# mosure/bevy_gaussian_splatting

Hardware: NVIDIA H100
Metric: rendered Msplats/sec @1080p, 6M-gaussian cloud (higher is better)
Workload: dtype f32 (f16-packed inputs)

## Files before the change

### bevy_gaussian_splatting_b200/csrc/project.cu

```cuda
#include <cuda_fp16.h>

#include "project_math.cuh"
#include "launch.cuh"

namespace bgs {

__constant__ float c_shc[16] = {
    0.28209479177387814f, -0.4886025119029199f, 0.4886025119029199f, -0.4886025119029199f,
    1.0925484305920792f, -1.0925484305920792f, 0.31539156525252005f, -1.0925484305920792f,
    0.5462742152960396f, -0.5900435899266435f, 2.890611442640554f, -0.4570457994644658f,
    0.3731763325901154f, -0.4570457994644658f, 1.445305721320277f, -0.5900435899266435f};

__device__ __forceinline__ void normalize3(const float a[3], float out[3]) {
    const float inv = rsqrtf((a[0] * a[0] + a[1] * a[1]) + a[2] * a[2]);
    out[0] = a[0] * inv; out[1] = a[1] * inv; out[2] = a[2] * inv;
}
__device__ __forceinline__ float dot3(const float a[3], const float b[3]) {
    return (a[0] * b[0] + a[1] * b[1]) + a[2] * b[2];
}
__device__ __forceinline__ float srgb_to_linear(float v) {
    if (v <= 0.04045f) return v * (1.0f / 12.92f);
    return __powf((v + 0.055f) * (1.0f / 1.055f), 2.4f);
}
__device__ __forceinline__ uint32_t pack_bbox(float lo, float hi) {
    return (uint32_t)(int)lo | ((uint32_t)(int)hi << 16);
}
constexpr uint32_t BBOX_EMPTY = 1u;

__device__ __forceinline__ void make_bbox(float cx, float cy, float hx, float hy, int Wi, int Hi,
                                          uint32_t& bx, uint32_t& by) {
    bx = BBOX_EMPTY; by = BBOX_EMPTY;
    if (!(hx >= 0.0f) || !(hy >= 0.0f) || !(cx == cx) || !(cy == cy)) return;
    const float sx = hx * 1.0e-3f + 1.0e-2f, sy = hy * 1.0e-3f + 1.0e-2f;
    float x0 = ceilf((cx - hx) - (0.5f + sx));
    float x1 = floorf((cx + hx) - (0.5f - sx));
    float y0 = ceilf((cy - hy) - (0.5f + sy));
    float y1 = floorf((cy + hy) - (0.5f - sy));
    if (!(x0 <= x1) || !(y0 <= y1)) return;
    x0 = fmaxf(x0, 0.0f); y0 = fmaxf(y0, 0.0f);
    x1 = fminf(x1, (float)(Wi - 1)); y1 = fminf(y1, (float)(Hi - 1));
    if (!(x0 <= x1) || !(y0 <= y1)) return;
    bx = pack_bbox(x0, x1); by = pack_bbox(y0, y1);
}

template <bool F16>
struct Attr;
template <>
struct Attr<false> {
    __device__ static float4 load(const void* blocks, uint32_t id, float* sh, float q[4], float so[4], bool need_sh,
                                  uint32_t* = nullptr) {
        const float4* b = reinterpret_cast<const float4*>(blocks) + (size_t)id * 16;
        const float4 p = __ldg(b), r = __ldg(b + 1), s = __ldg(b + 2);
        q[0] = r.x; q[1] = r.y; q[2] = r.z; q[3] = r.w;
        so[0] = s.x; so[1] = s.y; so[2] = s.z; so[3] = s.w;
        if (need_sh) {
#pragma unroll
            for (int i = 0; i < 12; ++i) {
                const float4 v = __ldg(b + 3 + i);
                sh[4 * i] = v.x; sh[4 * i + 1] = v.y; sh[4 * i + 2] = v.z; sh[4 * i + 3] = v.w;
            }
        }
        return p;
    }
};
template <>
struct Attr<true> {
    __device__ static float lo(uint32_t w) { return __half2float(__ushort_as_half((unsigned short)(w & 0xFFFFu))); }
    __device__ static float hi(uint32_t w) { return __half2float(__ushort_as_half((unsigned short)(w >> 16))); }
    __device__ static float4 load(const void* blocks, uint32_t id, float* sh, float q[4], float so[4], bool need_sh,
                                  uint32_t* op_bits = nullptr) {
        const uint4* b = reinterpret_cast<const uint4*>(blocks) + (size_t)id * 8;
        const uint4 pw = __ldg(b), w = __ldg(b + 1);
        if (op_bits) *op_bits = w.w & 0xFFFFu;
        q[0] = hi(w.x); q[1] = lo(w.x); q[2] = hi(w.y); q[3] = lo(w.y);
        so[0] = hi(w.z); so[1] = lo(w.z); so[2] = hi(w.w); so[3] = lo(w.w);
        if (need_sh) {
#pragma unroll
            for (int i = 0; i < 6; ++i) {
                const uint4 v = __ldg(b + 2 + i);
                sh[8 * i] = lo(v.x); sh[8 * i + 1] = hi(v.x); sh[8 * i + 2] = lo(v.y); sh[8 * i + 3] = hi(v.y);
                sh[8 * i + 4] = lo(v.z); sh[8 * i + 5] = hi(v.z); sh[8 * i + 6] = lo(v.w); sh[8 * i + 7] = hi(v.w);
            }
        }
        return make_float4(__uint_as_float(pw.x), __uint_as_float(pw.y), __uint_as_float(pw.z), __uint_as_float(pw.w));
    }
};

template <bool F16>
__global__ void repack_kernel(const uint4* __restrict__ pos, const uint4* __restrict__ sh, const uint4* __restrict__ rot,
                              const uint4* __restrict__ so, uint32_t n, uint4* __restrict__ blocks) {
    constexpr uint32_t CH = F16 ? 8u : 16u;
    constexpr uint32_t SHC = F16 ? 6u : 12u;
    const size_t i = (size_t)blockIdx.x * blockDim.x + threadIdx.x;
    if (i >= (size_t)n * CH) return;
    const uint32_t id = (uint32_t)(i / CH), c = (uint32_t)(i % CH);
    uint4 v = make_uint4(0u, 0u, 0u, 0u);
    if (c == 0) v = pos[id];
    else if (c == 1) v = rot[id];
    else if (!F16 && c == 2) v = so[id];
    else {
        const uint32_t k = c - (F16 ? 2u : 3u);
        if (k < SHC) v = sh[(size_t)id * SHC + k];
    }
    blocks[i] = v;
}
void launch_repack(bool f16, const void* pos, const void* sh, const void* rot, const void* so, uint32_t n, void* blocks,
                   cudaStream_t stream) {
    const size_t total = (size_t)n * (f16 ? 8 : 16);
    const uint32_t grid = (uint32_t)((total + 255) / 256);
    if (f16) repack_kernel<true><<<grid, 256, 0, stream>>>((const uint4*)pos, (const uint4*)sh, (const uint4*)rot, (const uint4*)so, n, (uint4*)blocks);
    else repack_kernel<false><<<grid, 256, 0, stream>>>((const uint4*)pos, (const uint4*)sh, (const uint4*)rot, (const uint4*)so, n, (uint4*)blocks);
}

__global__ void depth_range_kernel(const float4* __restrict__ pos, uint32_t n, const uint32_t* __restrict__ sorted_payload,
                                   const uint32_t* __restrict__ slot_ids ,
                                   FrameCounters* __restrict__ ctr, FrameConsts fc) {
    if (threadIdx.x != 0 || blockIdx.x != 0 || n < 2u) return;
    const uint32_t n_vis = ctr->n_vis, n_sorted = ctr->n_sort;
    auto id_at = [&](uint32_t i) { const uint32_t p = sorted_payload[i]; return slot_ids ? slot_ids[p] : p; };
    uint32_t first, last;
    if (n_sorted == n) {
        first = id_at(1u); last = id_at(n - 1u);
    } else {
        const uint32_t cmin = 0xFFFFFFFFu - ctr->culled_min_inv, cmax = ctr->culled_max_p1 - 1u;
        first = n_vis >= 2u ? id_at(1u) : cmin;
        last = (n - n_vis) >= 1u ? cmax : id_at(n - 1u);
    }
    auto dist = [&](uint32_t id) {
        const float4 p = pos[id];
        float pw[4];
        mat4_point(fc.model, p.x, p.y, p.z, pw);
        return sqrtf(cam_dist2(fc, pw));
    };
    ctr->depth_min = dist(last);
    ctr->depth_max = dist(first);
}

__device__ __forceinline__ float adaptive_cutoff(float opacity) {
    const float a = 9.0f + 2.0f * det_ln(opacity);
    return sqrtf(a > 0.000001f ? a : 0.000001f);
}
__global__ void cutoff_table_kernel(float* __restrict__ tab) {
    const uint32_t h = blockIdx.x * blockDim.x + threadIdx.x;
    if (h < 65536u) tab[h] = adaptive_cutoff(__half2float(__ushort_as_half((unsigned short)h)));
}
void launch_cutoff_table(float* tab, cudaStream_t stream) { cutoff_table_kernel<<<256, 256, 0, stream>>>(tab); }

template <bool F16>
__device__ __forceinline__ float splat_cutoff(const FrameConsts& fc, float opacity, const float* __restrict__ cutoff_tab,
                                              uint32_t op_bits) {
    if (!fc.adaptive) return 3.0f;
    if constexpr (F16) return __ldg(cutoff_tab + op_bits);
    else return adaptive_cutoff(opacity);
}

__device__ __forceinline__ void rotation_rows(const float q[4], float Rm[3][3]) {
    const float qr = q[0], x = q[1], y = q[2], z = q[3];
    Rm[0][0] = 1.0f - 2.0f * (y * y + z * z);
    Rm[1][0] = 2.0f * (x * y - qr * z);
    Rm[2][0] = 2.0f * (x * z + qr * y);
    Rm[0][1] = 2.0f * (x * y + qr * z);
    Rm[1][1] = 1.0f - 2.0f * (x * x + z * z);
    Rm[2][1] = 2.0f * (y * z - qr * x);
    Rm[0][2] = 2.0f * (x * z - qr * y);
    Rm[1][2] = 2.0f * (y * z + qr * x);
    Rm[2][2] = 1.0f - 2.0f * (x * x + y * y);
}

__device__ __forceinline__ void sigma3d(const FrameConsts& fc, const float A[3][3], const float Rm[3][3], const float sc[3],
                                        const float q[4], const float so[4], float c3[6]) {
    if (fc.cov_pre) {
        c3[0] = q[0]; c3[1] = q[1]; c3[2] = q[2]; c3[3] = q[3]; c3[4] = so[0]; c3[5] = so[1];
        return;
    }
    float M[3][3], Sg[3][3], X[3][3], TS[3][3];
#pragma unroll
    for (int i = 0; i < 3; ++i)
#pragma unroll
        for (int j = 0; j < 3; ++j) M[i][j] = sc[i] * Rm[i][j];
#pragma unroll
    for (int i = 0; i < 3; ++i)
#pragma unroll
        for (int j = 0; j < 3; ++j) Sg[i][j] = (M[0][i] * M[0][j] + M[1][i] * M[1][j]) + M[2][i] * M[2][j];
    const float mn = fminf(fminf(fminf(fabsf(Sg[0][0]), fabsf(Sg[0][1])), fminf(fabsf(Sg[0][2]), fabsf(Sg[1][1]))),
                           fminf(fabsf(Sg[1][2]), fabsf(Sg[2][2])));
    const float mx = fmaxf(fmaxf(fmaxf(fabsf(Sg[0][0]), fabsf(Sg[0][1])), fmaxf(fabsf(Sg[0][2]), fabsf(Sg[1][1]))),
                           fmaxf(fabsf(Sg[1][2]), fabsf(Sg[2][2])));
    if (fc.model_identity && mn > 0.0f && mx < __uint_as_float(0x7F800000u) && Sg[0][0] == Sg[0][0] &&
        Sg[0][1] == Sg[0][1] && Sg[0][2] == Sg[0][2] && Sg[1][1] == Sg[1][1] && Sg[1][2] == Sg[1][2] && Sg[2][2] == Sg[2][2]) {
#pragma unroll
        for (int i = 0; i < 3; ++i)
#pragma unroll
            for (int j = 0; j < 3; ++j) TS[i][j] = Sg[i][j];
    } else {
#pragma unroll
        for (int i = 0; i < 3; ++i)
#pragma unroll
            for (int j = 0; j < 3; ++j) X[i][j] = (A[i][0] * Sg[0][j] + A[i][1] * Sg[1][j]) + A[i][2] * Sg[2][j];
#pragma unroll
        for (int i = 0; i < 3; ++i)
#pragma unroll
            for (int j = 0; j < 3; ++j) TS[i][j] = (X[i][0] * A[j][0] + X[i][1] * A[j][1]) + X[i][2] * A[j][2];
    }
    c3[0] = TS[0][0]; c3[1] = TS[1][0]; c3[2] = TS[2][0]; c3[3] = TS[1][1]; c3[4] = TS[2][1]; c3[5] = TS[2][2];
}

struct Cov2d {
    float a, b, c, det, mid, term, l1;
};
__device__ __forceinline__ Cov2d cov2d(const FrameConsts& fc, const float pw[3], const float c3[6]) {
    const float Vrk[3][3] = {{c3[0], c3[1], c3[2]}, {c3[1], c3[3], c3[4]}, {c3[2], c3[4], c3[5]}};
    float tv[4];
    mat4_point(fc.view_from_world, pw[0], pw[1], pw[2], tv);
    const float fx = fc.p00 * fc.W, fy = fc.p11 * fc.H;
    const float sz = 1.0f / (tv[2] * tv[2]);
    const float J00 = fx / tv[2], J20 = -(fx * tv[0]) * sz;
    const float J11 = -fy / tv[2], J21 = (fy * tv[1]) * sz;
    float Tm[3][2];
#pragma unroll
    for (int i = 0; i < 3; ++i) {
        const float v0 = fc.view_from_world[i * 4 + 0], v1 = fc.view_from_world[i * 4 + 1],
                    v2 = fc.view_from_world[i * 4 + 2];
        Tm[i][0] = v0 * J00 + v2 * J20;
        Tm[i][1] = v1 * J11 + v2 * J21;
    }
    float Y[3][2];
#pragma unroll
    for (int i = 0; i < 3; ++i)
#pragma unroll
        for (int b = 0; b < 2; ++b) Y[i][b] = (Vrk[i][0] * Tm[0][b] + Vrk[i][1] * Tm[1][b]) + Vrk[i][2] * Tm[2][b];
    Cov2d v;
    v.a = ((Tm[0][0] * Y[0][0] + Tm[1][0] * Y[1][0]) + Tm[2][0] * Y[2][0]) + 0.3f;
    v.b = (Tm[0][1] * Y[0][0] + Tm[1][1] * Y[1][0]) + Tm[2][1] * Y[2][0];
    v.c = ((Tm[0][1] * Y[0][1] + Tm[1][1] * Y[1][1]) + Tm[2][1] * Y[2][1]) + 0.3f;
    v.det = v.a * v.c - v.b * v.b;
    v.mid = 0.5f * (v.a + v.c);
    v.term = sqrtf(fmaxf(0.0f, v.mid * v.mid - v.det));
    v.l1 = v.mid + v.term;
    return v;
}

__device__ __forceinline__ void aabb_record(const FrameConsts& fc, const Cov2d& v, float cutoff, SplatRec& rec) {
    const float l2 = fmaxf(v.mid - v.term, 0.0f);
    const float Rq = cutoff * fmaxf(sqrtf(v.l1), sqrtf(l2));
    const float dinv = 1.0f / v.det;
    rec.ux = v.c * dinv; rec.uy = -v.b * dinv; rec.vx = v.a * dinv; rec.vy = Rq;
    const float h = 0.5f * Rq;
    make_bbox(rec.cx, rec.cy, h, h, fc.Wi, fc.Hi, rec.bx, rec.by);
}

__device__ __forceinline__ void obb_record(const FrameConsts& fc, const Cov2d& v, float cutoff, SplatRec& rec) {
    const float a = v.a, b = v.b, c = v.c;
    const float aa = (a - c) * (a - c);
    const float bb = sqrtf(aa + (4.0f * b) * b);
    const float major = sqrtf(((a + c) + bb) * 0.5f);
    const float minor = sqrtf(((a + c) - bb) * 0.5f);
    const float Bx = cutoff * major, By = cutoff * minor;
    const float evx = -b, evy = v.l1 - a;
    const float el = sqrtf(evx * evx + evy * evy);
    const float e1x = evx / el, e1y = evy / el;
    const float e2x = e1y, e2y = -e1x;
    rec.ux = (2.0f * e1x) / Bx; rec.uy = (-2.0f * e1y) / Bx;
    rec.vx = (2.0f * e2x) / By; rec.vy = (-2.0f * e2y) / By;
    const float hx = 0.5f * (fabsf(e1x) * Bx + fabsf(e2x) * By);
    const float hy = 0.5f * (fabsf(e1y) * Bx + fabsf(e2y) * By);
    if (rec.ux == rec.ux && rec.uy == rec.uy && rec.vx == rec.vx && rec.vy == rec.vy)
        make_bbox(rec.cx, rec.cy, hx, hy, fc.Wi, fc.Hi, rec.bx, rec.by);
}

__device__ __forceinline__ void surfel_record(const FrameConsts& fc, const float A[3][3], const float Rm[3][3],
                                              const float sc[3], const float pw[3], float cutoff, uint32_t r,
                                              float4* __restrict__ extra, SplatRec& rec) {
    const float W = fc.W, H = fc.H;
    float L[3][2];
#pragma unroll
    for (int j = 0; j < 2; ++j) {
        const float rc[3] = {Rm[j][0] * sc[j], Rm[j][1] * sc[j], Rm[j][2] * sc[j]};
#pragma unroll
        for (int i = 0; i < 3; ++i) L[i][j] = (A[i][0] * rc[0] + A[i][1] * rc[1]) + A[i][2] * rc[2];
    }
    float G[3][4];
    mat4_dir(fc.clip_from_world, L[0][0], L[1][0], L[2][0], G[0]);
    mat4_dir(fc.clip_from_world, L[0][1], L[1][1], L[2][1], G[1]);
    mat4_point(fc.clip_from_world, pw[0], pw[1], pw[2], G[2]);
    const float fxk = fc.p00 * W / 2.0f, fyk = fc.p11 * H / 2.0f;
    const float cxk = (W - 1.0f) / 2.0f, cyk = (H - 1.0f) / 2.0f;
    float T0[3], T1[3], T2[3];
#pragma unroll
    for (int j = 0; j < 3; ++j) {
        T0[j] = fxk * G[j][0] + cxk * G[j][3];
        T1[j] = fyk * G[j][1] + cyk * G[j][3];
        T2[j] = G[j][3];
    }
    const float c2 = cutoff * cutoff;
    const float test[3] = {c2, c2, -1.0f};
    const float tt[3] = {test[0] * T2[0], test[1] * T2[1], test[2] * T2[2]};
    const float d = dot3(tt, T2);
    if (fabsf(d) < 1.0e-4f) return;
    const float inv = 1.0f / d;
    const float f[3] = {inv * test[0], inv * test[1], inv * test[2]};
    const float t02[3] = {T0[0] * T2[0], T0[1] * T2[1], T0[2] * T2[2]};
    const float t12[3] = {T1[0] * T2[0], T1[1] * T2[1], T1[2] * T2[2]};
    const float mean0 = dot3(f, t02), mean1 = dot3(f, t12);
    const float f0[3] = {f[0] * T0[0], f[1] * T0[1], f[2] * T0[2]};
    const float f1[3] = {f[0] * T1[0], f[1] * T1[1], f[2] * T1[2]};
    const float ex = mean0 * mean0 - dot3(f0, T0);
    const float ey = mean1 * mean1 - dot3(f1, T1);
    if (ex < 1.0e-4f || ey < 1.0e-4f) return;
    const float Rq = fmaxf(fmaxf(sqrtf(ex), sqrtf(ey)), cutoff * 0.707106f);
    rec.ux = 2.0f / Rq; rec.uy = 0.0f; rec.vx = 0.0f; rec.vy = -2.0f / Rq;
    const float h = 0.5f * Rq;
    if (Rq == Rq) make_bbox(rec.cx, rec.cy, h, h, fc.Wi, fc.Hi, rec.bx, rec.by);
    if (fc.aabb && extra != nullptr) {
        float4* e = extra + (size_t)r * 4;
        e[0] = make_float4(Rq, mean0, mean1, W / H);
        e[1] = make_float4(T0[0], T0[1], T0[2], 0.0f);
        e[2] = make_float4(T1[0], T1[1], T1[2], 0.0f);
        e[3] = make_float4(T2[0], T2[1], T2[2], 0.0f);
    }
}

__device__ __forceinline__ void sh_colour(const FrameConsts& fc, const float A[3][3], const float pw[3], const float sh[48],
                                          float rgb[3]) {
    const float dlt[3] = {pw[0] - fc.cam[0], pw[1] - fc.cam[1], pw[2] - fc.cam[2]};
    float dw[3], loc[3], dl[3];
    normalize3(dlt, dw);
    if (fc.model_identity) {
        loc[0] = dw[0]; loc[1] = dw[1]; loc[2] = dw[2];
    } else {
#pragma unroll
        for (int cc = 0; cc < 3; ++cc) {
            const float col[3] = {A[0][cc], A[1][cc], A[2][cc]};
            float bn[3];
            normalize3(col, bn);
            loc[cc] = dot3(bn, dw);
        }
    }
    normalize3(loc, dl);
    const float x = dl[0], y = dl[1], z = dl[2];
    const float xx = x * x, yy = y * y, zz = z * z;
    float basis[16];
    basis[0] = 1.0f;
    basis[1] = y; basis[2] = z; basis[3] = x;
    basis[4] = x * y; basis[5] = y * z; basis[6] = (2.0f * zz - xx) - yy;
    basis[7] = x * z; basis[8] = xx - yy;
    basis[9] = y * (3.0f * xx - yy);
    basis[10] = (x * y) * z;
    basis[11] = y * ((4.0f * zz - xx) - yy);
    basis[12] = z * ((2.0f * zz - 3.0f * xx) - 3.0f * yy);
    basis[13] = x * ((4.0f * zz - xx) - yy);
    basis[14] = z * (xx - yy);
    basis[15] = x * (xx - 3.0f * yy);
#pragma unroll
    for (int kk = 0; kk < 16; ++kk) basis[kk] *= c_shc[kk];
#pragma unroll
    for (int cc = 0; cc < 3; ++cc) {
        float acc = 0.5f;
#pragma unroll
        for (int kk = 0; kk < 16; ++kk) acc = fmaf(sh[3 * kk + cc], basis[kk], acc);
        rgb[cc] = acc;
    }
    if (fc.color_space == 0u) {
#pragma unroll
        for (int cc = 0; cc < 3; ++cc) rgb[cc] = srgb_to_linear(rgb[cc]);
    }
}

__device__ __forceinline__ void depth_colour(const FrameConsts& fc, const FrameCounters* __restrict__ ctr,
                                             const float pw[3], float rgb[3]) {
    if (fc.n_cloud < 2u) return;
    const float depth = sqrtf(cam_dist2(fc, pw));
    const float dmin = ctr->depth_min, dmax = ctr->depth_max;
    float nd = (depth - dmin) / (dmax - dmin);
    nd = fminf(fmaxf(nd, 0.0f), 1.0f);
    float t1 = (nd - 0.5f) / (1.0f - 0.5f); t1 = fminf(fmaxf(t1, 0.0f), 1.0f);
    float t2 = (nd - 0.0f) / (0.5f - 0.0f); t2 = fminf(fmaxf(t2, 0.0f), 1.0f);
    rgb[0] = t1 * t1 * (3.0f - 2.0f * t1);
    rgb[1] = 1.0f - fabsf(nd - 0.5f) * 2.0f;
    rgb[2] = 1.0f - t2 * t2 * (3.0f - 2.0f * t2);
}

__device__ __forceinline__ void normal_colour(const FrameConsts& fc, const float A[3][3], const float Rm[3][3],
                                              const float sc[3], float rgb[3]) {
    float SR[3], Ln[3], wn[4];
#pragma unroll
    for (int i = 0; i < 3; ++i) SR[i] = sc[i] * Rm[i][2];
#pragma unroll
    for (int i = 0; i < 3; ++i) Ln[i] = (A[i][0] * SR[0] + A[i][1] * SR[1]) + A[i][2] * SR[2];
    mat4_dir(fc.view_from_world, Ln[0], Ln[1], Ln[2], wn);
    const float l = sqrtf(((wn[0] * wn[0] + wn[1] * wn[1]) + wn[2] * wn[2]) + wn[3] * wn[3]);
#pragma unroll
    for (int cc = 0; cc < 3; ++cc) rgb[cc] = 0.5f * (wn[cc] / l + 1.0f);
}

__device__ __forceinline__ void position_colour(const FrameConsts& fc, const float pw[3], float rgb[3]) {
#pragma unroll
    for (int cc = 0; cc < 3; ++cc) rgb[cc] = (pw[cc] - fc.aabb_min[cc]) / (fc.aabb_max[cc] - fc.aabb_min[cc]);
}

constexpr float FRAC_PI_3_F = 1.0471975512f;
constexpr float PI_2_F = 6.28318530718f;

__device__ __forceinline__ void hsv_to_rgb(float h, float s, float v, float rgb[3]) {
    const float hk = h / FRAC_PI_3_F, vs = v * s;
    const float base[3] = {5.0f, 3.0f, 1.0f};
#pragma unroll
    for (int cc = 0; cc < 3; ++cc) {
        const float x = base[cc] + hk;
        const float k = x - 6.0f * truncf(x / 6.0f);
        rgb[cc] = v - vs * fmaxf(0.0f, fminf(k, fminf(4.0f - k, 1.0f)));
    }
}

__device__ __forceinline__ float det_atan2(float yf, float xf) {
    if (yf != yf || xf != xf) return __uint_as_float(0x7FC00000u);
    const double ay = fabs((double)yf), ax = fabs((double)xf);
    const bool steep = ay > ax;
    double t;
    if (ax == ay) t = ax == 0.0 ? 0.0 : 1.0;
    else t = steep ? __ddiv_rn(ax, ay) : __ddiv_rn(ay, ax);
    double base = 0.0, u = t;
    if (t > 0.41421356237309503) { base = 0.7853981633974483; u = __ddiv_rn(__dsub_rn(t, 1.0), __dadd_rn(t, 1.0)); }
    const double z = __dmul_rn(u, u);
    double p = -1.0 / 43.0;
#pragma unroll
    for (int k = 20; k >= 0; --k) p = __dadd_rn(__dmul_rn(p, z), (k & 1 ? -1.0 : 1.0) / (double)(2 * k + 1));
    double r = __dadd_rn(base, __dmul_rn(u, p));
    if (steep) r = __dsub_rn(1.5707963267948966, r);
    if (__float_as_uint(xf) >> 31) r = __dsub_rn(3.141592653589793, r);
    if (__float_as_uint(yf) >> 31) r = -r;
    return (float)r;
}

__device__ __forceinline__ void class_colour(const ModeConsts& mc, float vis, float rgb[3]) {
    if (vis < 2.0f) return;
    const float hue = ((vis - 2.0f) / (float)mc.num_classes) * 6.283185307f;
    float h[3];
    hsv_to_rgb(hue, 1.0f, 1.0f, h);
#pragma unroll
    for (int cc = 0; cc < 3; ++cc) rgb[cc] = rgb[cc] * (1.0f - 0.5f) + h[cc] * 0.5f;
}

__device__ __forceinline__ void flow_colour(const FrameConsts& fc, const ModeConsts& mc, const float pw[3], float rgb[3]) {
    float c[4], cp[4];
    mat4_point(fc.clip_from_world, pw[0], pw[1], pw[2], c);
    mat4_point(mc.prev_clip_from_world, pw[0], pw[1], pw[2], cp);
    const float mvx = (c[0] / c[3] - cp[0] / cp[3]) * 0.5f;
    const float mvy = (c[1] / c[3] - cp[1] / cp[3]) * -0.5f;
    const float fx = mvx / mc.delta_time, fy = mvy / mc.delta_time;
    const float radius = sqrtf(fx * fx + fy * fy);
    float angle = det_atan2(fy, fx);
    if (angle < 0.0f) angle = angle + PI_2_F;
    hsv_to_rgb(angle, fminf(fmaxf(radius, 0.0f), 1.0f), 1.0f, rgb);
}

__device__ __forceinline__ void highlight_selected(SplatRec& rec, float drgb[3], float nrgb[3]) {
    rec.r = 0.3f; rec.g = 1.0f; rec.b = 0.1f; rec.op = 1.0f;
    drgb[0] = nrgb[0] = 0.3f; drgb[1] = nrgb[1] = 1.0f; drgb[2] = nrgb[2] = 0.1f;
}

__device__ __forceinline__ void store_rec(SplatRec* __restrict__ dst, const SplatRec& rec) {
    float4* out = reinterpret_cast<float4*>(dst);
    out[0] = make_float4(rec.cx, rec.cy, rec.ux, rec.uy);
    out[1] = make_float4(rec.vx, rec.vy, __uint_as_float(rec.bx), __uint_as_float(rec.by));
    out[2] = make_float4(rec.r, rec.g, rec.b, rec.op);
}

template <bool F16, bool MODES2>
__device__ __forceinline__ void project_one(const FrameConsts& fc, const FrameCounters* __restrict__ ctr, uint32_t r,
                                            float4 p4, const float q[4], const float so[4], const float sh[48],
                                            const float* __restrict__ cutoff_tab, uint32_t op_bits,
                                            SplatRec* __restrict__ recs, float4* __restrict__ extra,
                                            float4* __restrict__ aux, const ModeConsts& mc) {
    SplatRec rec;
    rec.ux = 0.f; rec.uy = 0.f; rec.vx = 0.f; rec.vy = 0.f;
    rec.bx = BBOX_EMPTY; rec.by = BBOX_EMPTY;
    rec.r = 0.f; rec.g = 0.f; rec.b = 0.f;
    float pw[4], ndc[2];
    mat4_point(fc.model, p4.x, p4.y, p4.z, pw);
    const bool visible = in_frustum(fc, pw, ndc);
    const float hw = 0.5f * fc.W, hh = 0.5f * fc.H;
    rec.cx = ndc[0] * hw + hw;
    rec.cy = hh - ndc[1] * hh;
    const float opacity = so[3];
    rec.op = opacity * fc.global_opacity;
    if (visible && !(fc.draw_mode == BGS_DRAW_SELECTED && p4.w < 0.5f)) {
        const float cutoff = splat_cutoff<F16>(fc, opacity, cutoff_tab, op_bits);
        float A[3][3], Rm[3][3];
#pragma unroll
        for (int rr = 0; rr < 3; ++rr)
#pragma unroll
            for (int cc = 0; cc < 3; ++cc) A[rr][cc] = fc.model[cc * 4 + rr];
        rotation_rows(q, Rm);
        const float sc[3] = {so[0] * fc.global_scale, so[1] * fc.global_scale, so[2] * fc.global_scale};

        if (fc.gaussian_mode == BGS_GAUSSIAN_3D) {
            float c3[6];
            sigma3d(fc, A, Rm, sc, q, so, c3);
            const Cov2d v = cov2d(fc, pw, c3);
            if (fc.aabb) aabb_record(fc, v, cutoff, rec);
            else obb_record(fc, v, cutoff, rec);
        } else {
            surfel_record(fc, A, Rm, sc, pw, cutoff, r, extra, rec);
        }

        const uint32_t mode = fc.rasterize_mode;
        float rgb[3] = {0.f, 0.f, 0.f}, drgb[3] = {0.f, 0.f, 0.f}, nrgb[3] = {0.f, 0.f, 0.f};
        if constexpr (MODES2) {
            if (mode == BGS_RASTERIZE_CLASSIFICATION) {
                sh_colour(fc, A, pw, sh, rgb);
                class_colour(mc, p4.w, rgb);
            } else {
                flow_colour(fc, mc, pw, rgb);
            }
            rec.r = rgb[0]; rec.g = rgb[1]; rec.b = rgb[2];
        } else {
            if (mode == BGS_RASTERIZE_COLOR) sh_colour(fc, A, pw, sh, rgb);
            if (mode == BGS_RASTERIZE_POSITION) position_colour(fc, pw, rgb);
            if (mode == BGS_RASTERIZE_DEPTH || fc.aux) depth_colour(fc, ctr, pw, drgb);
            if (mode == BGS_RASTERIZE_NORMAL || fc.aux) normal_colour(fc, A, Rm, sc, nrgb);
            const bool depth = mode == BGS_RASTERIZE_DEPTH, normal = mode == BGS_RASTERIZE_NORMAL;
            rec.r = depth ? drgb[0] : normal ? nrgb[0] : rgb[0];
            rec.g = depth ? drgb[1] : normal ? nrgb[1] : rgb[1];
            rec.b = depth ? drgb[2] : normal ? nrgb[2] : rgb[2];
        }
        if (fc.draw_mode == BGS_DRAW_HIGHLIGHT_SELECTED && p4.w > 0.5f) highlight_selected(rec, drgb, nrgb);
        if (fc.aux && aux != nullptr) {
            aux[(size_t)r * 2] = make_float4(drgb[0], drgb[1], drgb[2], 0.0f);
            aux[(size_t)r * 2 + 1] = make_float4(nrgb[0], nrgb[1], nrgb[2], 0.0f);
        }
    }
    store_rec(recs + r, rec);
}

constexpr int PROJ_MIN_CTAS = 6;
template <bool F16>
__global__ void __launch_bounds__(128, PROJ_MIN_CTAS)
project_kernel(const void* __restrict__ blocks, const uint32_t* __restrict__ index_list, int by_slot,
               const FrameCounters* __restrict__ ctr, FrameConsts fc, SplatRec* __restrict__ recs,
               float4* __restrict__ extra , const float* __restrict__ cutoff_tab,
               float4* __restrict__ aux ) {
    const uint32_t n_vis = ctr->n_vis;
    for (uint32_t r = blockIdx.x * blockDim.x + threadIdx.x; r < n_vis; r += gridDim.x * blockDim.x) {
        const uint32_t id = by_slot ? __ldg(index_list + r) : __ldg(index_list + (n_vis - 1u - r));
        float sh[48], q[4], so[4];
        const bool need_sh = fc.rasterize_mode == BGS_RASTERIZE_COLOR;
        uint32_t op_bits = 0u;
        const float4 p4 = Attr<F16>::load(blocks, id, sh, q, so, need_sh, &op_bits);
        project_one<F16, false>(fc, ctr, r, p4, q, so, sh, cutoff_tab, op_bits, recs, extra, aux, ModeConsts{});
    }
}

template <bool F16>
__global__ void __launch_bounds__(128, PROJ_MIN_CTAS)
project_modes_kernel(const void* __restrict__ blocks, const uint32_t* __restrict__ index_list, int by_slot,
                     const FrameCounters* __restrict__ ctr, FrameConsts fc, ModeConsts mc, SplatRec* __restrict__ recs,
                     float4* __restrict__ extra, const float* __restrict__ cutoff_tab) {
    const uint32_t n_vis = ctr->n_vis;
    for (uint32_t r = blockIdx.x * blockDim.x + threadIdx.x; r < n_vis; r += gridDim.x * blockDim.x) {
        const uint32_t id = by_slot ? __ldg(index_list + r) : __ldg(index_list + (n_vis - 1u - r));
        float sh[48], q[4], so[4];
        const bool need_sh = fc.rasterize_mode == BGS_RASTERIZE_CLASSIFICATION;
        uint32_t op_bits = 0u;
        const float4 p4 = Attr<F16>::load(blocks, id, sh, q, so, need_sh, &op_bits);
        project_one<F16, true>(fc, ctr, r, p4, q, so, sh, cutoff_tab, op_bits, recs, extra, nullptr, mc);
    }
}

void launch_depth_range(const float4* pos, uint32_t n, const uint32_t* sorted_payload, const uint32_t* slot_ids,
                        FrameCounters* ctr, const FrameConsts& fc, cudaStream_t stream) {
    depth_range_kernel<<<1, 32, 0, stream>>>(pos, n, sorted_payload, slot_ids, ctr, fc);
}

void launch_project(bool f16, const void* blocks, const uint32_t* index_list, int by_slot, const FrameCounters* ctr,
                    const FrameConsts& fc, SplatRec* recs, float4* extra, uint32_t n_hint, int sm_count,
                    const float* cutoff_tab, float4* aux, const ModeConsts* modes, cudaStream_t stream) {
    uint32_t grid = (n_hint + 127) / 128;
    if (grid > 65535u * 8u) grid = 65535u * 8u;
    if (grid < (uint32_t)sm_count) grid = (uint32_t)sm_count;
    if (modes) {
        if (f16) project_modes_kernel<true><<<grid, 128, 0, stream>>>(blocks, index_list, by_slot, ctr, fc, *modes, recs, extra, cutoff_tab);
        else project_modes_kernel<false><<<grid, 128, 0, stream>>>(blocks, index_list, by_slot, ctr, fc, *modes, recs, extra, cutoff_tab);
        return;
    }
    if (f16) project_kernel<true><<<grid, 128, 0, stream>>>(blocks, index_list, by_slot, ctr, fc, recs, extra, cutoff_tab, aux);
    else project_kernel<false><<<grid, 128, 0, stream>>>(blocks, index_list, by_slot, ctr, fc, recs, extra, cutoff_tab, aux);
}

}
```

Baseline: 16430.

## Warp-cooperative cp.async gather of splat attribute blocks with double buffering

Result: faster. 17230, median of 6 (+4.9%).

```diff
diff --git a/bevy_gaussian_splatting_b200/csrc/project.cu b/bevy_gaussian_splatting_b200/csrc/project.cu
--- a/bevy_gaussian_splatting_b200/csrc/project.cu
+++ b/bevy_gaussian_splatting_b200/csrc/project.cu
@@ -43,20 +43,43 @@
     bx = pack_bbox(x0, x1); by = pack_bbox(y0, y1);
 }
 
+__device__ __forceinline__ void cp_async16(uint4* dst_shared, const uint4* src) {
+    asm volatile("cp.async.cg.shared.global [%0], [%1], 16;" ::"r"((uint32_t)__cvta_generic_to_shared(dst_shared)), "l"(src)
+                 : "memory");
+}
+__device__ __forceinline__ void cp_async_commit() { asm volatile("cp.async.commit_group;" ::: "memory"); }
+template <int N>
+__device__ __forceinline__ void cp_async_wait() { asm volatile("cp.async.wait_group %0;" ::"n"(N) : "memory"); }
+
+template <int CH, int NP>
+__device__ __forceinline__ void gather_blocks(const uint4* __restrict__ blocks, uint32_t id, uint32_t n_valid,
+                                              uint4* stage, int lane) {
+    static_assert(32 % NP == 0 && NP <= CH, "NP lanes per block");
+#pragma unroll
+    for (int k = 0; k < NP; ++k) {
+        const int g = (32 * k + lane) / NP, p = lane % NP;
+        const uint32_t gid = __shfl_sync(0xFFFFFFFFu, id, g);
+        if ((uint32_t)g < n_valid) cp_async16(stage + g * CH + (p ^ (g & 7)), blocks + (size_t)gid * CH + p);
+    }
+}
+
 template <bool F16>
 struct Attr;
 template <>
 struct Attr<false> {
-    __device__ static float4 load(const void* blocks, uint32_t id, float* sh, float q[4], float so[4], bool need_sh,
-                                  uint32_t* = nullptr) {
-        const float4* b = reinterpret_cast<const float4*>(blocks) + (size_t)id * 16;
-        const float4 p = __ldg(b), r = __ldg(b + 1), s = __ldg(b + 2);
+    static constexpr int CH = 16, GEO = 4;
+    __device__ static float4 load(const uint4* stage, int g, float* sh, float q[4], float so[4], bool need_sh, uint32_t&) {
+        auto piece = [&](int p) {
+            const uint4 v = stage[g * CH + (p ^ (g & 7))];
+            return make_float4(__uint_as_float(v.x), __uint_as_float(v.y), __uint_as_float(v.z), __uint_as_float(v.w));
+        };
+        const float4 p = piece(0), r = piece(1), s = piece(2);
         q[0] = r.x; q[1] = r.y; q[2] = r.z; q[3] = r.w;
         so[0] = s.x; so[1] = s.y; so[2] = s.z; so[3] = s.w;
         if (need_sh) {
 #pragma unroll
             for (int i = 0; i < 12; ++i) {
-                const float4 v = __ldg(b + 3 + i);
+                const float4 v = piece(3 + i);
                 sh[4 * i] = v.x; sh[4 * i + 1] = v.y; sh[4 * i + 2] = v.z; sh[4 * i + 3] = v.w;
             }
         }
@@ -65,19 +88,20 @@
 };
 template <>
 struct Attr<true> {
+    static constexpr int CH = 8, GEO = 2;
     __device__ static float lo(uint32_t w) { return __half2float(__ushort_as_half((unsigned short)(w & 0xFFFFu))); }
     __device__ static float hi(uint32_t w) { return __half2float(__ushort_as_half((unsigned short)(w >> 16))); }
-    __device__ static float4 load(const void* blocks, uint32_t id, float* sh, float q[4], float so[4], bool need_sh,
-                                  uint32_t* op_bits = nullptr) {
-        const uint4* b = reinterpret_cast<const uint4*>(blocks) + (size_t)id * 8;
-        const uint4 pw = __ldg(b), w = __ldg(b + 1);
-        if (op_bits) *op_bits = w.w & 0xFFFFu;
+    __device__ static float4 load(const uint4* stage, int g, float* sh, float q[4], float so[4], bool need_sh,
+                                  uint32_t& op_bits) {
+        auto piece = [&](int p) { return stage[g * CH + (p ^ (g & 7))]; };
+        const uint4 pw = piece(0), w = piece(1);
+        op_bits = w.w & 0xFFFFu;
         q[0] = hi(w.x); q[1] = lo(w.x); q[2] = hi(w.y); q[3] = lo(w.y);
         so[0] = hi(w.z); so[1] = lo(w.z); so[2] = hi(w.w); so[3] = lo(w.w);
         if (need_sh) {
 #pragma unroll
             for (int i = 0; i < 6; ++i) {
-                const uint4 v = __ldg(b + 2 + i);
+                const uint4 v = piece(2 + i);
                 sh[8 * i] = lo(v.x); sh[8 * i + 1] = hi(v.x); sh[8 * i + 2] = lo(v.y); sh[8 * i + 3] = hi(v.y);
                 sh[8 * i + 4] = lo(v.z); sh[8 * i + 5] = hi(v.z); sh[8 * i + 6] = lo(v.w); sh[8 * i + 7] = hi(v.w);
             }
@@ -533,38 +557,64 @@
     store_rec(recs + r, rec);
 }
 
-constexpr int PROJ_MIN_CTAS = 6;
+constexpr int PROJ_THREADS = 128, PROJ_WARPS = PROJ_THREADS / 32, PROJ_MIN_CTAS = 4;
+
+template <bool F16, bool MODES2>
+__device__ __forceinline__ void project_groups(const void* __restrict__ blocks, const uint32_t* __restrict__ index_list,
+                                               int by_slot, const FrameCounters* __restrict__ ctr, const FrameConsts& fc,
+                                               bool need_sh, SplatRec* __restrict__ recs, float4* __restrict__ extra,
+                                               const float* __restrict__ cutoff_tab, float4* __restrict__ aux,
+                                               const ModeConsts& mc) {
+    constexpr int CH = Attr<F16>::CH;
+    __shared__ __align__(16) uint4 s_stages[PROJ_WARPS][32 * CH];
+    const int lane = threadIdx.x & 31;
+    uint4* const stage = s_stages[threadIdx.x >> 5];
+    const uint32_t n_vis = ctr->n_vis, stride = gridDim.x * PROJ_THREADS;
+    auto list_id = [&](uint32_t r) {
+        return r < n_vis ? (by_slot ? __ldg(index_list + r) : __ldg(index_list + (n_vis - 1u - r))) : 0u;
+    };
+    auto gather = [&](uint32_t r0, uint32_t id) {
+        const uint32_t n_valid = r0 < n_vis ? n_vis - r0 : 0u;
+        const uint4* b = reinterpret_cast<const uint4*>(blocks);
+        if (need_sh) gather_blocks<CH, CH>(b, id, n_valid, stage, lane);
+        else gather_blocks<CH, Attr<F16>::GEO>(b, id, n_valid, stage, lane);
+        cp_async_commit();
+    };
+    uint32_t r0 = (blockIdx.x * PROJ_WARPS + (threadIdx.x >> 5)) * 32u;
+    gather(r0, list_id(r0 + lane));
+    uint32_t id_next = list_id(r0 + stride + lane);
+    for (; r0 < n_vis; r0 += stride) {
+        cp_async_wait<0>();
+        __syncwarp();
+        const uint32_t r = r0 + lane;
+        float sh[48], q[4], so[4];
+        uint32_t op_bits = 0u;
+        float4 p4 = make_float4(0.f, 0.f, 0.f, 0.f);
+        if (r < n_vis) p4 = Attr<F16>::load(stage, lane, sh, q, so, need_sh, op_bits);
+        __syncwarp();
+        gather(r0 + stride, id_next);
+        id_next = list_id(r0 + 2u * stride + lane);
+        if (r < n_vis) project_one<F16, MODES2>(fc, ctr, r, p4, q, so, sh, cutoff_tab, op_bits, recs, extra, aux, mc);
+    }
+}
+
 template <bool F16>
-__global__ void __launch_bounds__(128, PROJ_MIN_CTAS)
+__global__ void __launch_bounds__(PROJ_THREADS, PROJ_MIN_CTAS)
 project_kernel(const void* __restrict__ blocks, const uint32_t* __restrict__ index_list, int by_slot,
                const FrameCounters* __restrict__ ctr, FrameConsts fc, SplatRec* __restrict__ recs,
                float4* __restrict__ extra , const float* __restrict__ cutoff_tab,
                float4* __restrict__ aux ) {
-    const uint32_t n_vis = ctr->n_vis;
-    for (uint32_t r = blockIdx.x * blockDim.x + threadIdx.x; r < n_vis; r += gridDim.x * blockDim.x) {
-        const uint32_t id = by_slot ? __ldg(index_list + r) : __ldg(index_list + (n_vis - 1u - r));
-        float sh[48], q[4], so[4];
-        const bool need_sh = fc.rasterize_mode == BGS_RASTERIZE_COLOR;
-        uint32_t op_bits = 0u;
-        const float4 p4 = Attr<F16>::load(blocks, id, sh, q, so, need_sh, &op_bits);
-        project_one<F16, false>(fc, ctr, r, p4, q, so, sh, cutoff_tab, op_bits, recs, extra, aux, ModeConsts{});
-    }
+    project_groups<F16, false>(blocks, index_list, by_slot, ctr, fc, fc.rasterize_mode == BGS_RASTERIZE_COLOR, recs, extra,
+                               cutoff_tab, aux, ModeConsts{});
 }
 
 template <bool F16>
-__global__ void __launch_bounds__(128, PROJ_MIN_CTAS)
+__global__ void __launch_bounds__(PROJ_THREADS, PROJ_MIN_CTAS)
 project_modes_kernel(const void* __restrict__ blocks, const uint32_t* __restrict__ index_list, int by_slot,
                      const FrameCounters* __restrict__ ctr, FrameConsts fc, ModeConsts mc, SplatRec* __restrict__ recs,
                      float4* __restrict__ extra, const float* __restrict__ cutoff_tab) {
-    const uint32_t n_vis = ctr->n_vis;
-    for (uint32_t r = blockIdx.x * blockDim.x + threadIdx.x; r < n_vis; r += gridDim.x * blockDim.x) {
-        const uint32_t id = by_slot ? __ldg(index_list + r) : __ldg(index_list + (n_vis - 1u - r));
-        float sh[48], q[4], so[4];
-        const bool need_sh = fc.rasterize_mode == BGS_RASTERIZE_CLASSIFICATION;
-        uint32_t op_bits = 0u;
-        const float4 p4 = Attr<F16>::load(blocks, id, sh, q, so, need_sh, &op_bits);
-        project_one<F16, true>(fc, ctr, r, p4, q, so, sh, cutoff_tab, op_bits, recs, extra, nullptr, mc);
-    }
+    project_groups<F16, true>(blocks, index_list, by_slot, ctr, fc, fc.rasterize_mode == BGS_RASTERIZE_CLASSIFICATION, recs,
+                              extra, cutoff_tab, nullptr, mc);
 }
 
 void launch_depth_range(const float4* pos, uint32_t n, const uint32_t* sorted_payload, const uint32_t* slot_ids,
@@ -575,16 +625,16 @@
 void launch_project(bool f16, const void* blocks, const uint32_t* index_list, int by_slot, const FrameCounters* ctr,
                     const FrameConsts& fc, SplatRec* recs, float4* extra, uint32_t n_hint, int sm_count,
                     const float* cutoff_tab, float4* aux, const ModeConsts* modes, cudaStream_t stream) {
-    uint32_t grid = (n_hint + 127) / 128;
-    if (grid > 65535u * 8u) grid = 65535u * 8u;
-    if (grid < (uint32_t)sm_count) grid = (uint32_t)sm_count;
+    uint32_t grid = (n_hint + PROJ_THREADS - 1) / PROJ_THREADS;
+    if (grid > (uint32_t)(PROJ_MIN_CTAS * sm_count)) grid = (uint32_t)(PROJ_MIN_CTAS * sm_count);
+    if (grid < 1u) grid = 1u;
     if (modes) {
-        if (f16) project_modes_kernel<true><<<grid, 128, 0, stream>>>(blocks, index_list, by_slot, ctr, fc, *modes, recs, extra, cutoff_tab);
-        else project_modes_kernel<false><<<grid, 128, 0, stream>>>(blocks, index_list, by_slot, ctr, fc, *modes, recs, extra, cutoff_tab);
+        if (f16) project_modes_kernel<true><<<grid, PROJ_THREADS, 0, stream>>>(blocks, index_list, by_slot, ctr, fc, *modes, recs, extra, cutoff_tab);
+        else project_modes_kernel<false><<<grid, PROJ_THREADS, 0, stream>>>(blocks, index_list, by_slot, ctr, fc, *modes, recs, extra, cutoff_tab);
         return;
     }
-    if (f16) project_kernel<true><<<grid, 128, 0, stream>>>(blocks, index_list, by_slot, ctr, fc, recs, extra, cutoff_tab, aux);
-    else project_kernel<false><<<grid, 128, 0, stream>>>(blocks, index_list, by_slot, ctr, fc, recs, extra, cutoff_tab, aux);
-}
-
-}
+    if (f16) project_kernel<true><<<grid, PROJ_THREADS, 0, stream>>>(blocks, index_list, by_slot, ctr, fc, recs, extra, cutoff_tab, aux);
+    else project_kernel<false><<<grid, PROJ_THREADS, 0, stream>>>(blocks, index_list, by_slot, ctr, fc, recs, extra, cutoff_tab, aux);
+}
+
+}
```
